# hjr37/diff-gaussian-rasterization

Hardware: AMD Instinct MI355X
Metric: Mviews/sec fwd+bwd @1080p, 500k Gaussians (higher is better)
Workload: dtype f32

## Files before the change

### diff-gaussian-rasterization_amd/csrc/api.hip

```cpp
#include <hip/hip_runtime.h>

#include <algorithm>
#include <string>

#include "../../include/dgr_hip.h"
#include "dgr_common.h"
#include "host_util.h"
#include "kernels.h"
#include "options.h"
#include "profile.h"
#include "status.h"

namespace dgr {
namespace {
thread_local std::string g_last_error = "";
}
void set_last_error(const std::string& text) { g_last_error = text; }
}

using namespace dgr;

namespace {

struct FwdCommon {
// ... 108 lines not shown
    return DGR_OK;
}

template <class A>
void blend_fwd_common(A& r, const FwdCommon& c, dgr::GeometryView geom, dgr::ImageView img, dgr::BinningView bin, ArmedReport* armed) {
    r.W = c.W; r.H = c.H; r.grid_x = dgr::tiles_x(c.W); r.grid_y = dgr::tiles_y(c.H);
    r.sched = img.tile_sched; r.ranges = img.ranges; r.sched_flag = img.cursor + 3; r.point_list = bin.point_list; r.rec = geom.rec; r.bg = c.background;
    r.out_color = c.out_color; r.out_depth = c.out_depth; r.n_contrib = img.n_contrib; r.status = img.status;
    r.rep = armed ? armed->rep : dgr::StatusReport{nullptr, 0u, nullptr};
}
int forward_blend(const FwdCommon& c, dgr::GeometryView geom, dgr::ImageView img, dgr::BinningView bin, hipStream_t st, bool full,
                  ArmedReport* armed = nullptr) {
    ScopedStage t(ST_RENDER_FWD, st);
    if (full) {
        dgr::RenderFwdFullArgs r{};
        blend_fwd_common(r, c, geom, img, bin, armed);
        r.out_uncertainty = c.out_alpha; r.n_valid = img.n_valid; r.first_contrib = img.first_contrib; r.final_T = img.final_T;
        HIP_TRY(dgr::launch_render_fwd_full(r, opt_alpha_mode(), st));
    } else {
        dgr::RenderFwdLightArgs r{};
        blend_fwd_common(r, c, geom, img, bin, armed);
        r.gt_depth = c.gt_depth; r.out_median = c.out_median_depth; r.out_alpha = c.out_alpha; r.out_depth_var = c.out_depth_var;
        r.gau_uncertainty = c.gau_uncertainty; r.gau_related_pixels = c.gau_related_pixels;
        HIP_TRY(dgr::launch_render_fwd_light(r, opt_alpha_mode(), st));
    }
    if (armed) armed->handed_over = true;
    return DGR_OK;
}

int check_common(const FwdCommon& c) {
    if (c.P < 0 || c.W <= 0 || c.H <= 0) { set_last_error("bad sizes"); return DGR_ERR_BAD_ARGUMENT; }
    if ((unsigned)c.P > DGR_ID_MASK) { set_last_error("more than 2^28 Gaussians"); return DGR_ERR_BAD_ARGUMENT; }
    if (c.P > 0 && !c.shs && !c.colors_precomp) { set_last_error("need SHs or precomputed colours"); return DGR_ERR_BAD_ARGUMENT; }
    if (c.P > 0 && !c.cov3D_precomp && (!c.scales || !c.rotations)) { set_last_error("need scale/rotation or cov3D"); return DGR_ERR_BAD_ARGUMENT; }
    if (dgr::tiles_x(c.W) > 65535 || dgr::tiles_y(c.H) > 65535 || (long long)c.W * c.H > (1ll << 30)) { set_last_error("image too large"); return DGR_ERR_BAD_ARGUMENT; }
    return DGR_OK;
}

inline int batch_stream_count(int n_views) {
    const int kmax = std::max(1, std::min(option(OPT_BATCH_STREAMS), DGR_BATCH_MAX_STREAMS));
    const int rounds = (n_views + kmax - 1) / kmax;
    return (n_views + rounds - 1) / rounds;
}
struct BatchStreams {
    int device = -1;
    hipStream_t helper[DGR_BATCH_MAX_STREAMS - 1] = {};
// ... 267 lines not shown
    s.ds = DetScratch{nullptr, nullptr, nullptr, 0};
    if (!scratch_clean) { ScopedStage t(ST_ZERO, st); HIP_TRY(dgr::launch_zero_fill(s.sc.acc, s.sc.zero_bytes, st)); }
    if (w.dL_dmean2D_abs) { ScopedStage t(ST_ZERO, st); HIP_TRY(dgr::launch_zero_floats(w.dL_dmean2D_abs, 3 * (size_t)P, st)); }
    if (det) {
        s.ds = carve_det_scratch(w.scratch, P, w.R);
        { ScopedStage t(ST_ZERO, st); HIP_TRY(dgr::launch_zero_fill(s.ds.rows, sizeof(float) * DGR_ACC_STRIDE * (size_t)w.R, st)); }
        HIP_TRY(dgr::launch_det_offsets(P, s.geom.rect, s.ds.blk, s.geom.goff, st));
    }
    return DGR_OK;
}

template <class A>
void blend_bwd_common(A& r, const BwdView& w, const float* bg, int W, int H, const BwdBufs& s, bool det) {
    r.W = W; r.H = H; r.grid_x = dgr::tiles_x(W); r.grid_y = dgr::tiles_y(H);
    r.sched = s.img.tile_sched; r.ranges = s.img.ranges; r.sched_flag = s.img.cursor + 3; r.point_list = (const uint32_t*)w.binning_buffer;
    r.rec = s.geom.rec; r.bg = bg; r.gt_depth = w.gt_depth; r.n_contrib = s.img.n_contrib; r.acc = s.sc.acc;
    if (det) { r.det_rows = s.ds.rows; r.det_rect = s.geom.rect; r.det_goff = s.geom.goff; r.det_R = (uint32_t)w.R; }
}
int blend_bwd_light(const BwdView& w, const dgr::PreprocessBwdArgs& b, const float* bg, const BwdBufs& s, bool det, bool complete,
                    hipStream_t st) {
    dgr::RenderBwdLightArgs r{};
    blend_bwd_common(r, w, bg, b.W, b.H, s, det);
    r.alphas = w.alphas; r.dL_dpix = w.dL_dpix; r.dL_dpix_depth = w.dL_dpix_depth; r.dL_dpix_median = w.dL_dpix_median_depth;
    r.dL_dpix_var = w.dL_dpix_depth_var; r.dL_dpix_silhouette = w.dL_dpix_silhouette;
    r.means3D = b.means3D; r.view = w.viewmatrix; r.track_off = b.track_off; r.map_off = complete ? 0 : b.map_off;
    ScopedStage t(ST_RENDER_BWD, st);
    if (w.dL_dmean2D_abs) HIP_TRY(dgr::launch_render_bwd_light_abs(r, w.dL_dmean2D_abs, opt_alpha_mode(), st));
    else HIP_TRY(dgr::launch_render_bwd_light(r, opt_alpha_mode(), st));
    return DGR_OK;
}
int blend_bwd_full(const BwdView& w, const dgr::PreprocessBwdArgs& b, const float* bg, const BwdBufs& s, bool det, hipStream_t st) {
    dgr::RenderBwdFullArgs r{};
    blend_bwd_common(r, w, bg, b.W, b.H, s, det);
    r.final_T = s.img.final_T; r.first_contrib = s.img.first_contrib;
    r.dL_dpix = w.dL_dpix; r.dL_depths = w.dL_depths; r.dL_duncertainties = w.dL_duncertainties;
    r.dL_dpix_silhouette = w.dL_dpix_silhouette;
    ScopedStage t(ST_RENDER_BWD, st);
    if (w.dL_dmean2D_abs) HIP_TRY(dgr::launch_render_bwd_full_abs(r, w.dL_dmean2D_abs, opt_alpha_mode(), st));
    else HIP_TRY(dgr::launch_render_bwd_full(r, opt_alpha_mode(), st, det));
    return DGR_OK;
}
int bwd_view_blend(const BwdView& w, const dgr::PreprocessBwdArgs& b, const float* bg, const BwdBufs& s, bool det, bool complete,
                   hipStream_t st) {
    const int rc = b.full_variant ? blend_bwd_full(w, b, bg, s, det, st) : blend_bwd_light(w, b, bg, s, det, complete, st);
    if (rc) return rc;
    if (det) HIP_TRY(dgr::launch_det_gather(b.P, s.geom.rect, s.geom.goff, s.ds.rows, (uint32_t)w.R, s.sc.acc, st));
    return DGR_OK;
// ... 534 lines not shown
```

### diff-gaussian-rasterization_amd/csrc/kernels.h

```cpp
#pragma once
#include <hip/hip_ext.h>
#include "dgr_common.h"

namespace dgr {

struct LaunchEvents {
    hipEvent_t start, stop;
    bool used;
};
extern thread_local LaunchEvents* g_launch_events;

template <typename K, typename... Args>
inline void launch(K kernel, dim3 grid, dim3 block, hipStream_t stream, Args... args) {
    LaunchEvents* ev = g_launch_events;
    if (ev && !ev->used) {
        ev->used = true;
        hipExtLaunchKernelGGL(kernel, grid, block, 0, stream, ev->start, ev->stop, 0, args...);
    } else {
        hipLaunchKernelGGL(kernel, grid, block, 0, stream, args...);
    }
}
template <typename K, typename... Args>
inline void launch_shmem(K kernel, dim3 grid, dim3 block, size_t shmem, hipStream_t stream, Args... args) {
    LaunchEvents* ev = g_launch_events;
// ... 110 lines not shown
    double* det_pose;
};
struct PreprocessBwdBatchArgs {
    PreprocessBwdArgs base;
    int V;
    BwdViewPart v[DGR_MAX_BATCH_VIEWS];
};

struct RenderFwdLightArgs {
    int W, H, grid_x, grid_y;
    const uint4* sched;
    const uint2* ranges;
    const uint32_t* sched_flag;
    uint32_t* point_list;
    const float4* rec;
    const float* bg;
    const float* gt_depth;
    float* out_color;
    float* out_depth;
    float* out_median;
    float* out_alpha;
    float* out_depth_var;
    uint32_t* n_contrib;
    float* gau_uncertainty;
    int* gau_related_pixels;
    StatusReport rep;
    const int* status;
};

struct RenderBwdLightArgs {
    int W, H, grid_x, grid_y;
    const uint4* sched;
    const uint2* ranges;
    const uint32_t* sched_flag;
    const uint32_t* point_list;
    const float4* rec;
    const float* bg;
    const float* gt_depth;
    const float* alphas;
    const uint32_t* n_contrib;
    const float* dL_dpix;
    const float* dL_dpix_depth;
    const float* dL_dpix_median;
    const float* dL_dpix_var;
    const float* dL_dpix_silhouette;
    const float* means3D;
    const float* view;
    float* acc;
    int track_off, map_off;
    float* det_rows;
    const ushort4* det_rect;
    const uint32_t* det_goff;
    uint32_t det_R;
};

struct RenderFwdFullArgs {
    int W, H, grid_x, grid_y;
    const uint4* sched;
    const uint2* ranges;
    const uint32_t* sched_flag;
    uint32_t* point_list;
    const float4* rec;
    const float* bg;
// ... 93 lines not shown
```

### diff-gaussian-rasterization_amd/csrc/render_common.h

```cpp
#pragma once
#include "dgr_common.h"
#include "kernels.h"
#include "wave_reduce.h"
#include "exact_math.h"

namespace dgr {

__device__ __forceinline__ uint4 blend_slot(const uint4* __restrict__ sched, const uint2* __restrict__ ranges,
                                            const uint32_t* __restrict__ sched_flag, int tiles, bool* overflowed = nullptr,
                                            bool* quadrant_lists = nullptr) {
    const int flag = __builtin_amdgcn_readfirstlane((int)*sched_flag);
    if (overflowed) *overflowed = (flag & 2) != 0;
    if (quadrant_lists) *quadrant_lists = (flag & 4) != 0;
    if (flag & 1) return sched[blockIdx.x];
    const int tile = xcd_contiguous((int)blockIdx.x, tiles);
    const uint2 r = ranges[tile];
    return make_uint4((uint32_t)tile, r.x, r.y, 0u);
}

__device__ __forceinline__ bool wave_any(bool p) { return __builtin_amdgcn_ballot_w64(p) != 0ull; }

namespace {

constexpr float LOG2E = 1.4426950408889634f, LN2 = 0.6931471805599453f;
// ... 6 lines not shown
    static constexpr float PSCALE = LOG2 ? LOG2E : 1.0f;
    static constexpr float PUNSCALE = LOG2 ? LN2 : 1.0f;
    static constexpr bool TABLE = (AM == ALPHA_GLIBC);
};
template <int AM, bool UNTESTED_ARG = false>
__device__ __forceinline__ float alpha_raw(float o, float p2, const uint64_t* tab) {
    if (AM == ALPHA_FAST) return o * __builtin_amdgcn_exp2f(p2);
    if (AM == ALPHA_GLIBC) return o * exp_glibc<UNTESTED_ARG>(p2, tab);
    return o * exp_p32<UNTESTED_ARG>(p2);
}
template <int AM>
__device__ __forceinline__ float t_div(float T, float om, float& inv) {
    if (AM == ALPHA_FAST) { inv = __builtin_amdgcn_rcpf(om); return T * inv; }
    return div_ref(T, om, inv);
}

template <int NB, typename LIST_T = unsigned short, int NLISTS = 4, bool KEEP_ID = true>
struct StagedT {
    typedef LIST_T list_t;
    static constexpr bool HAS_ID = KEEP_ID;
    static constexpr int SLOTS = NB;
    static constexpr int SENTINEL = NB;
    static constexpr int LIST_LD = NB + 8;
    float4 rec[2 * (NB + 1)];
    float4 rgbd[NB + 1];
    uint32_t id[KEEP_ID ? NB : 1];
    LIST_T list[NLISTS][LIST_LD];
    int cnt4[4][NLISTS];
};
using Staged = StagedT<DGR_TILE_PIX>;

template <bool HALF_CODES>
__device__ __forceinline__ unsigned reach_code(const float4& q0, const float4& q1, float l2, float tile_x0, float tile_y0);

template <int AM, bool HALF_CODES = false, class S>
__device__ __forceinline__ unsigned stage_one(S& s, int slot, uint32_t gid, const float4* __restrict__ rec,
                                              float tile_x0, float tile_y0) {
    const float4 q0 = rec[DGR_REC_STRIDE * (size_t)gid + 0];
    const float4 q1 = rec[DGR_REC_STRIDE * (size_t)gid + 1];
    const float4 q2 = rec[DGR_REC_STRIDE * (size_t)gid + 2];
    const float o = q0.w;
    const float l2 = __log2f(o * (255.0f / 15.0f));
    constexpr float PSCALE = AlphaPath<AM>::PSCALE;
    float lthr = (o > 0.f) ? (-l2 * (AlphaPath<AM>::LOG2 ? 1.0f : LN2) - 1.0e-4f) : 3.0e38f;
    float zword = __int_as_float(slot);
    if (HALF_CODES) {
// ... 42 lines not shown
}

__device__ __forceinline__ uint32_t pack4(uint32_t w) { return (w & 1u) | ((w >> 7) & 2u) | ((w >> 14) & 4u) | ((w >> 21) & 8u); }
__device__ __forceinline__ uint32_t tag_byte(uint32_t up, uint32_t lo) { return spread4(pack4(up)) | (spread4(pack4(lo)) << 1); }

template <int AM, int TAGS, class S>
__device__ __forceinline__ unsigned stage_tagged(S& s, int slot, uint32_t entry, const float4* __restrict__ rec,
                                                 const uint8_t* __restrict__ tag8) {
    constexpr float PSCALE = AlphaPath<AM>::PSCALE;
    unsigned code = (unsigned)*tag8;
    if (code == 0u) return 0u;
    if (TAGS == TAGS_BYTES_QUADRANT) code = fold8(code);
    const uint32_t gid = entry & ID_MASK;
    const float4 q0 = rec[DGR_REC_STRIDE * (size_t)gid + 0];
    const float4 q1 = rec[DGR_REC_STRIDE * (size_t)gid + 1];
    const float4 q2 = rec[DGR_REC_STRIDE * (size_t)gid + 2];
    s.rec[2 * slot] = make_float4(q0.x, q0.y, -0.5f * PSCALE * q1.x, -0.5f * PSCALE * q1.z);
    s.rec[2 * slot + 1] = make_float4(-PSCALE * q1.y, q0.w, __int_as_float(slot * 4), __int_as_float(slot * 16));
    s.rgbd[slot] = make_float4(q2.x, q2.y, q2.z, q0.z);
    s.id[slot] = gid;
    return code;
}

__device__ __forceinline__ int lanes_below(unsigned long long m) {
    return (int)__builtin_amdgcn_mbcnt_hi((unsigned)(m >> 32), __builtin_amdgcn_mbcnt_lo((unsigned)m, 0u));
}

template <class S>
__device__ __forceinline__ int build_lists(S& s, unsigned code, int tid, int wave, int lane) {
    typedef typename S::list_t LT;
    unsigned long long bal[4];
#pragma unroll
    for (int w = 0; w < 4; w++) {
        bal[w] = __ballot((code >> w) & 1u);
        if (lane == 0) s.cnt4[wave][w] = __popcll(bal[w]);
    }
    __syncthreads();
#pragma unroll
    for (int w = 0; w < 4; w++) {
        if ((code >> w) & 1u) {
            int base = 0;
            for (int sw = 0; sw < wave; sw++) base += s.cnt4[sw][w];
            s.list[w][base + lanes_below(bal[w])] = (LT)(tid * 32);
        }
    }
    const int n = __builtin_amdgcn_readfirstlane(s.cnt4[0][wave] + s.cnt4[1][wave] + s.cnt4[2][wave] + s.cnt4[3][wave]);
    __syncthreads();
    if (lane < 4) s.list[wave][n + lane] = (LT)(S::SENTINEL * 32);
    return n;
}

template <class S>
__device__ __forceinline__ int build_half_lists(S& s, unsigned code, int tid, int wave, int lane) {
    typedef typename S::list_t LT;
    unsigned long long bal[8];
#pragma unroll
    for (int l = 0; l < 8; l++) {
        bal[l] = __ballot((code >> l) & 1u);
        if (lane == 0) s.cnt4[wave][l] = __popcll(bal[l]);
    }
    __syncthreads();
    int before = 0, all = 0;
    if (lane < 8) {
#pragma unroll
        for (int sw = 0; sw < 4; sw++) {
            const int c = s.cnt4[sw][lane];
            before += sw < wave ? c : 0;
            all += c;
        }
    }
#pragma unroll
    for (int l = 0; l < 8; l++) {
        const int base = __builtin_amdgcn_readlane(before, l);
        if ((code >> l) & 1u) s.list[l][base + lanes_below(bal[l])] = (LT)(tid * 32);
    }
    const int l0 = 2 * wave;
    const int n0 = __builtin_amdgcn_readlane(all, l0), n1 = __builtin_amdgcn_readlane(all, l0 + 1);
    __syncthreads();
    const int n = max(n0, n1);
    for (int i = n0 + lane; i < n + 4; i += 64) s.list[l0][i] = (LT)(S::SENTINEL * 32);
    for (int i = n1 + lane; i < n + 4; i += 64) s.list[l0 + 1][i] = (LT)(S::SENTINEL * 32);
    return n;
}

template <class S>
__device__ __forceinline__ int build_paired_lists(S& s, unsigned code8, int tid, int wave, int lane, unsigned long long (&split)[2]) {
    typedef typename S::list_t LT;
    static_assert(sizeof(LT) == 4 && S::SLOTS <= 128, "paired lists: 32-bit entries, at most two ranks per lane");
    unsigned long long bal[4];
#pragma unroll
    for (int w = 0; w < 4; w++) {
        bal[w] = __ballot(((code8 >> (2 * w)) & 3u) != 0u);
        if (lane == 0) s.cnt4[wave][w] = __popcll(bal[w]);
    }
    __syncthreads();
    int before = 0, all = 0;
    if (lane < 4) {
#pragma unroll
        for (int sw = 0; sw < 4; sw++) {
            const int c = s.cnt4[sw][lane];
            before += sw < wave ? c : 0;
            all += c;
        }
    }
#pragma unroll
    for (int w = 0; w < 4; w++) {
        const unsigned t = (code8 >> (2 * w)) & 3u;
        const int base = __builtin_amdgcn_readlane(before, w);
        if (t != 0u) s.list[2 * w][base + lanes_below(bal[w])] = (LT)(tid * 32) | t;
    }
    const int n = __builtin_amdgcn_readlane(all, wave);
    __syncthreads();
    LT* const LU = s.list[2 * wave];
    LT* const LL = s.list[2 * wave + 1];
    if (n <= 64) {
        const bool have = lane < n;
        const unsigned e0 = have ? LU[lane] : 0u;
        const int t0 = (int)(e0 & 3u);
        const int tm1 = __builtin_amdgcn_update_dpp(0, t0, 0x138, 0xf, 0xf, true);
        const int tm2 = __builtin_amdgcn_update_dpp(0, tm1, 0x138, 0xf, 0xf, true);
        const int tp1 = __builtin_amdgcn_update_dpp(0, t0, 0x130, 0xf, 0xf, true);
        const int tp2 = __builtin_amdgcn_update_dpp(0, tp1, 0x130, 0xf, 0xf, true);
        const bool odd = (lane & 1) != 0;
        const bool a_self = odd ? (tm1 * t0 == 2) : (t0 * tp1 == 2);
        const bool a_side = odd ? (tp1 * tp2 == 2) : (tm2 * tm1 == 2);
        const bool p2 = !a_self && !a_side && (odd ? (t0 * tp1 == 2) : (tm1 * t0 == 2));
        const bool first = odd ? p2 : a_self, second = odd ? a_self : p2;
        const unsigned long long keep = __ballot(have && !second);
        const int steps = __popcll(keep);
        if (have) {
            const int st = lanes_below(keep) - (second ? 1 : 0);
            const LT o = e0 & ~3u;
            if (first || second) {
                (t0 == 1 ? LU : LL)[st] = o;
            } else {
                LU[st] = o;
                LL[st] = o;
            }
        }
        if (lane < 4) {
            LU[steps + lane] = (LT)(S::SENTINEL * 32);
            LL[steps + lane] = (LT)(S::SENTINEL * 32);
        }
        split[0] = __ballot(lane < steps && LU[lane] != LL[lane]);
        split[1] = 0ull;
        return steps;
    }
    const LT ea = lane < n ? LU[lane] : 0u, eb = lane + 64 < n ? LU[lane + 64] : 0u;
    if (lane < n) { LU[lane] = ea & ~3u; LL[lane] = ea & ~3u; }
    if (lane + 64 < n) { LU[lane + 64] = eb & ~3u; LL[lane + 64] = eb & ~3u; }
    if (lane < 4) {
        LU[n + lane] = (LT)(S::SENTINEL * 32);
        LL[n + lane] = (LT)(S::SENTINEL * 32);
    }
    split[0] = split[1] = 0ull;
    return n;
}

typedef float f2 __attribute__((ext_vector_type(2)));

template <int AM>
__device__ __forceinline__ float pair_p2(const float4& q0, const float4& q1, f2 pxy, f2& dxy) {
    const f2 g = {q0.x, q0.y}, ac = {q0.z, q0.w};
    dxy = g - pxy;
    if (AM == ALPHA_FAST) {
        const f2 m = ac * dxy;
        const float t = __builtin_fmaf(q1.x, dxy.y, m.x);
        return __builtin_fmaf(dxy.x, t, m.y * dxy.y);
    } else {
#pragma clang fp contract(off)
        const f2 m = (ac * dxy) * dxy;
        const float B = (q1.x * dxy.x) * dxy.y;
        return (m.x + m.y) + B;
    }
}

// ... 47 lines not shown
```

### diff-gaussian-rasterization_amd/csrc/render_light.hip

```cpp
#include "render_common.h"

namespace dgr {
namespace {

constexpr int FWD_UNROLL = 2;

template <bool HALVES>
struct StagedFwd {
    typedef StagedT<DGR_TILE_PIX, unsigned short, HALVES ? 8 : 4, !HALVES> staged_t;
    staged_t f;
    float unc[DGR_TILE_PIX];
    uint32_t cnt[DGR_TILE_PIX];
    uint32_t hit[DGR_TILE_PIX];
    uint64_t exptab[32];
};


template <class SF>
__device__ __forceinline__ void flush_slot(const SF& sf, const RenderFwdLightArgs& a, uint8_t* tag8, uint32_t pos0, int tid, bool staged) {
    if (!staged) return;
    uint32_t t8;
    if constexpr (!SF::staged_t::HAS_ID) {
        t8 = tag_byte(sf.hit[tid], __float_as_uint(sf.f.rec[2 * tid + 1].z));
    } else {
        t8 = spread4(pack4(sf.hit[tid])) * 3u;
    }
    tag8[pos0 + tid] = (uint8_t)t8;
    if (sf.cnt[tid] != 0u) {
        uint32_t gid;
        if constexpr (SF::staged_t::HAS_ID) gid = sf.f.id[tid];
        else gid = a.point_list[pos0 + tid];
        atomicAdd(&a.gau_uncertainty[gid], sf.unc[tid]);
        atomicAdd(&a.gau_related_pixels[gid], (int)sf.cnt[tid]);
    }
}

template <int AM, bool HALVES>
__device__ __forceinline__ void render_fwd_light_body(const RenderFwdLightArgs& a, StagedFwd<HALVES>& sf, const uint4 slot, const bool overflowed) {
    typename StagedFwd<HALVES>::staged_t& s = sf.f;
    const int tile = (int)slot.x;
    const int tx = tile % a.grid_x, ty = tile / a.grid_x;
    const int tid = threadIdx.x, wave = tid >> 6, lane = tid & 63;
    const int px = tx * DGR_BLOCK_X + (wave & 1) * 8 + (lane & 7);
    const int py = ty * DGR_BLOCK_Y + (wave >> 1) * 8 + (lane >> 3);
    const bool inside = px < a.W && py < a.H;
    const uint32_t pix_id = (uint32_t)a.W * (uint32_t)py + (uint32_t)px;
    const f2 pxy = {(float)px, (float)py};
    const float tile_x0 = (float)(tx * DGR_BLOCK_X), tile_y0 = (float)(ty * DGR_BLOCK_Y);
    const int my_list = HALVES ? 2 * wave + (lane >> 5) : wave;
    uint8_t* const tag8 = half_tags(a.point_list, a.sched_flag);
    unsigned char* const mark_base = (HALVES && lane >= 32) ? reinterpret_cast<unsigned char*>(&s.rec[1].z) + wave
                                                             : reinterpret_cast<unsigned char*>(sf.hit) + wave;
    const int mark_stride = (HALVES && lane >= 32) ? 32 : 4;

    const uint2 range = make_uint2(slot.y, slot.z);
    const int total = (int)(range.y - range.x);

    float T = 1.0f, C0 = 0.f, C1 = 0.f, C2 = 0.f, weight = 0.f, Dd = 0.f, D_median = 0.f;
    uint32_t last_contributor = 0;
    float ub = inside ? 0.f : -__builtin_inff();
    const float gt_px = inside ? a.gt_depth[pix_id] : 0.f;
    if (tid == 0) write_sentinel(s);
    if (AlphaPath<AM>::TABLE) exp_ref_table_fill(sf.exptab, tid);
    bool have_flush = false;
    int last_base = 0;

    for (int base = 0; base < total; base += DGR_TILE_PIX) {
        if (__syncthreads_and(ub < 0.f)) break;
        last_base = base;
        if (have_flush) flush_slot(sf, a, tag8, range.x + base - DGR_TILE_PIX, tid, true);
        sf.unc[tid] = 0.f;
        sf.cnt[tid] = 0u;
        sf.hit[tid] = 0u;
        have_flush = true;
        const int cnt = min(DGR_TILE_PIX, total - base);
        unsigned code = 0;
        if (tid < cnt) code = stage_one<AM, HALVES>(s, tid, a.point_list[range.x + base + tid], a.rec, tile_x0, tile_y0);
        const int n = HALVES ? build_half_lists(s, code, tid, wave, lane) : build_lists(s, code, tid, wave, lane);

        for (int k = 0; k < n; k += FWD_UNROLL) {
            float4 q0[FWD_UNROLL], q1[FWD_UNROLL];
            load2(s, my_list, k, q0, q1);
#pragma unroll
            for (int u = 0; u < FWD_UNROLL; u++) {
                f2 dxy;
                const float p2 = pair_p2<AM>(q0[u], q1[u], pxy, dxy);
                if ((p2 <= ub) & (p2 >= q1[u].w)) {
                  const float alpha = fminf(0.99f, alpha_raw<AM>(q1[u].y, p2, sf.exptab));
                  if (alpha >= ALPHA_MIN) {
#pragma clang fp contract(off)
                    const float test_T = T * (1.0f - alpha);
                    if (test_T < 0.0001f) {
                        ub = -__builtin_inff();
// ... 1 lines not shown
                        const int j = HALVES ? (__float_as_int(q1[u].w) & 0xFF) : __float_as_int(q1[u].z);
                        const float4 cd = s.rgbd[j];
                        mark_base[j * mark_stride] = 1;
                        const float w = alpha * T;
                        C0 = __builtin_fmaf(cd.x, w, C0); C1 = __builtin_fmaf(cd.y, w, C1); C2 = __builtin_fmaf(cd.z, w, C2);
                        weight = weight + w;
                        Dd = __builtin_fmaf(cd.w, w, Dd);
                        if (T > 0.5f && test_T < 0.5f) {
                            D_median = cd.w;
                            const float e = cd.w - gt_px;
                            atomicAdd(&sf.unc[j], e * e * w);
                            atomicAdd(&sf.cnt[j], 1u);
                        }
                        T = test_T;
                        last_contributor = (uint32_t)(base + j + 1);
                    }
                  }
                }
            }
            if (!wave_any(ub >= 0.f)) break;
        }
    }
    __syncthreads();
    if (have_flush) flush_slot(sf, a, tag8, range.x + last_base, tid, tid < total - last_base);
    for (int p = (have_flush ? last_base + DGR_TILE_PIX : 0) + tid; p < total; p += DGR_TILE_PIX) tag8[range.x + p] = 0;

    if (overflowed) {
        C0 = C1 = C2 = weight = Dd = D_median = __builtin_nanf("");
    }
    if (inside) {
        const uint32_t N = (uint32_t)a.W * (uint32_t)a.H;
        a.n_contrib[pix_id] = last_contributor;
        a.out_color[pix_id] = C0 + T * a.bg[0];
        a.out_color[N + pix_id] = C1 + T * a.bg[1];
        a.out_color[2 * N + pix_id] = C2 + T * a.bg[2];
        a.out_alpha[pix_id] = weight;
        a.out_depth[pix_id] = Dd;
        a.out_median[pix_id] = D_median;
        a.out_depth_var[pix_id] = 0.0f;
    }
}

template <int AM>
__global__ void __launch_bounds__(256, 8) render_fwd_light_kernel(RenderFwdLightArgs a) {
    __shared__ union { StagedFwd<true> h; StagedFwd<false> q; } sf;
    if (a.rep.host && blockIdx.x == 0 && threadIdx.x == 0) report_status(a.rep, a.status);
    bool overflowed, quadrant_lists;
    const uint4 slot = blend_slot(a.sched, a.ranges, a.sched_flag, a.grid_x * a.grid_y, &overflowed, &quadrant_lists);
    if (quadrant_lists) render_fwd_light_body<AM, false>(a, sf.q, slot, overflowed);
    else render_fwd_light_body<AM, true>(a, sf.h, slot, overflowed);
}

constexpr int NACC_LIGHT = 14;

template <bool DET, bool HALVES = false, bool ABS = false>
struct StagedBwd {
    static constexpr int NB = DET ? 64 : 128;
    static constexpr int LD = NB + 1;
    static constexpr int PLANE = NACC_LIGHT * LD;
    static constexpr int NACC = ABS ? NACC_LIGHT + 2 : NACC_LIGHT;
    typedef StagedT<NB, uint32_t, HALVES ? 8 : 4> staged_t;
    staged_t f;
    float acc[(DET ? 4 : 1) * PLANE + (ABS ? 2 * LD : 0)];
    uint32_t inst[DET ? NB : 1];
    int max_last;
    uint64_t exptab[32];
};

template <int AM, bool DO_MAP, bool DO_POSE, bool DET, bool LEAN, bool HALVES, bool ABS = false>
__device__ __forceinline__ void render_bwd_light_body(const RenderBwdLightArgs& a, StagedBwd<DET, HALVES, ABS>& sb, const uint4 slot,
                                                      float* __restrict__ abs_out = nullptr) {
    static_assert(!HALVES || !DET, "half-wave / paired lists: not with the deterministic kernel's planes (LDS)");
    static_assert(!ABS || (DO_MAP && !DET), "absgrad: the mapping backward, not the deterministic kernel");
    constexpr bool PAIRED = HALVES && DO_MAP;
    typedef StagedBwd<DET, HALVES, ABS> SB;
    constexpr int BWD_NB = SB::NB, BWD_LD = SB::LD;
    typename SB::staged_t& s = sb.f;
    const int tile = (int)slot.x;
    const int tx = tile % a.grid_x, ty = tile / a.grid_x;
    const int tid = threadIdx.x, wave = tid >> 6, lane = tid & 63;
    const int px = tx * DGR_BLOCK_X + (wave & 1) * 8 + (lane & 7);
    const int py = ty * DGR_BLOCK_Y + (wave >> 1) * 8 + (lane >> 3);
    const bool inside = px < a.W && py < a.H;
    const uint32_t pix_id = (uint32_t)a.W * (uint32_t)py + (uint32_t)px;
    const uint32_t N = (uint32_t)a.W * (uint32_t)a.H;
    const float pxf = (float)px, pyf = (float)py;
    const f2 pxy = {pxf, pyf};

    const uint2 range = make_uint2(slot.y, slot.z);
    const int last_contributor = inside ? (int)a.n_contrib[pix_id] : 0;

    if (tid == 0) {
        sb.max_last = 0;
        write_sentinel<true>(s);
    }
    if (AlphaPath<AM>::TABLE) exp_ref_table_fill(sb.exptab, tid);
    __syncthreads();
    {
        int v = last_contributor;
#pragma unroll
        for (int off = 32; off > 0; off >>= 1) v = max(v, __shfl_xor(v, off, 64));
        if (lane == 0) atomicMax(&sb.max_last, v);
    }
    __syncthreads();
    const int total = min((int)(range.y - range.x), sb.max_last);
    if (total <= 0) return;

    const float T_final = inside ? (1.0f - a.alphas[pix_id]) : 0.f;
    float T = T_final;
    float dpix0 = 0.f, dpix1 = 0.f, dpix2 = 0.f, dpix_depth = 0.f, dpix_median = 0.f, dpix_var = 0.f, gt_px = 0.f, dpix_sil = 0.f;
    if (inside) {
        dpix0 = __builtin_nontemporal_load(a.dL_dpix + pix_id);
        dpix1 = __builtin_nontemporal_load(a.dL_dpix + N + pix_id);
        dpix2 = __builtin_nontemporal_load(a.dL_dpix + 2 * N + pix_id);
        dpix_depth = __builtin_nontemporal_load(a.dL_dpix_depth + pix_id);
        if (a.dL_dpix_silhouette) dpix_sil = __builtin_nontemporal_load(a.dL_dpix_silhouette + pix_id);
        if (!LEAN) {
            if (a.dL_dpix_median) dpix_median = __builtin_nontemporal_load(a.dL_dpix_median + pix_id);
            if (a.dL_dpix_var) dpix_var = __builtin_nontemporal_load(a.dL_dpix_var + pix_id);
            gt_px = __builtin_nontemporal_load(a.gt_depth + pix_id);
        }
    }
    const float bg_term = -T_final * ((a.bg[0] * dpix0 + a.bg[1] * dpix1 + a.bg[2] * dpix2) - dpix_sil);
    const float ddelx_dx = 0.5f * a.W, ddely_dy = 0.5f * a.H;
    float S = 0.f;
    float mid_thr = 0.5f;
    int my_comp;
    if (DO_MAP) {
        const int c = (lane >= 48) ? 12 : wave_reduce12d_comp(lane);
        my_comp = ((lane & 3) != 0 || c > 11) ? -1 : (c == 10 ? (DO_POSE ? 13 : 10) : c == 11 ? (DO_POSE ? 10 : -1) : c);
    } else if (HALVES) {
        const int c = half_reduce3_comp(lane);
        my_comp = c == 0 ? 4 : c == 1 ? 5 : c == 2 ? 13 : -1;
    } else {
        const int c = wave_reduce4_comp(lane);
        my_comp = ((lane & 15) == 0 && c < 3) ? (c == 0 ? 4 : c == 1 ? 5 : 13) : -1;
    }
    const int my_list = HALVES ? 2 * wave + (lane >> 5) : wave;
    const uint8_t* const tag8 = half_tags(a.point_list, a.sched_flag);

    float* const my_acc = sb.acc + (DET ? wave * SB::PLANE : 0) + (my_comp >= 0 ? my_comp : 0) * BWD_LD;

    for (int hi = total; hi > 0; hi -= BWD_NB) {
        const int lo = max(0, hi - BWD_NB);
        const int cnt = hi - lo;
        __syncthreads();
        unsigned code = 0;
        if (tid < cnt) code = stage_tagged<AM, HALVES ? TAGS_BYTES_HALVES : TAGS_BYTES_QUADRANT>(s, tid, a.point_list[range.x + lo + tid], a.rec, tag8 + (range.x + lo + tid));
        if (!DET) {
#pragma unroll
            for (int k = 0; k < SB::NACC; k++)
                if (BWD_NB == DGR_TILE_PIX || tid < BWD_NB) sb.acc[k * BWD_LD + tid] = 0.f;
        }
        unsigned long long split[2] = {0ull, 0ull};
        const int n = PAIRED   ? build_paired_lists(s, code, tid, wave, lane, split)
                      : HALVES ? build_half_lists(s, code, tid, wave, lane)
                               : build_lists(s, code, tid, wave, lane);
        const int rel_last4 = 4 * (last_contributor - lo);

        constexpr int U = PAIRED ? 1 : 2;
        for (int k = ((n + U - 1) / U) * U - U; k >= 0; k -= U) {
            float4 q0[2], q1[2];
            if (U == 2) {
                load2(s, my_list, k, q0, q1);
            } else {
                const unsigned off = s.list[my_list][k];
                q0[0] = *reinterpret_cast<const float4*>(reinterpret_cast<const char*>(s.rec) + off);
                q1[0] = *reinterpret_cast<const float4*>(reinterpret_cast<const char*>(s.rec) + off + 16);
            }
#pragma unroll
            for (int u = U - 1; u >= 0; u--) {
                f2 dxy;
                const float p2 = pair_p2<AM>(q0[u], q1[u], pxy, dxy);
                const float dx = dxy.x, dy = dxy.y;
                const int j4 = __float_as_int(q1[u].z);
                const float oG = alpha_raw<AM, true>(q1[u].y, p2, sb.exptab);
                const bool valid = (j4 < rel_last4) & (p2 <= 0.0f) & !(oG < ALPHA_MIN);
                const float oGm = valid ? oG : 0.f;
                const float alpha = fminf(0.99f, oGm);
                const float4 cd = *reinterpret_cast<const float4*>(reinterpret_cast<const char*>(s.rgbd) + __float_as_int(q1[u].w));
                const float om = 1.f - alpha;
                float inv;
                T = t_div<AM>(T, om, inv);
                const float w = alpha * T;
                const float e = cd.w - gt_px;
                const float X = LEAN ? cd.x * dpix0 + cd.y * dpix1 + cd.z * dpix2 + cd.w * dpix_depth
                                     : cd.x * dpix0 + cd.y * dpix1 + cd.z * dpix2 + cd.w * dpix_depth + (e * e) * dpix_var;
                const float dL_dalpha = (X - S) * T + bg_term * inv;
                S = alpha * X + om * S;
                const float qq = oGm * dL_dalpha;
                const float qdx = qq * dx, qdy = qq * dy;
                const float wd = w * dpix_depth;
                float tot;
                if (DO_MAP) {
                    float gmed = 0.f;
                    if (!LEAN) {
                        const bool fire = valid & (T > mid_thr);
                        gmed = fire ? dpix_median : 0.f;
                        mid_thr = fire ? __builtin_inff() : mid_thr;
                    }
                    float g[12];
                    g[0] = w * dpix0;
                    g[1] = w * dpix1;
// ... 51 lines not shown
        if (DET && tid < BWD_NB) {
            uint32_t row = ~0u;
            if (code != 0u) {
#pragma unroll
                for (int k = 0; k < NACC_LIGHT; k++) {
                    const bool delivered = DO_MAP ? (k <= 9 || k == 10 || (DO_POSE && k == 13)) : (k == 4 || k == 5 || k == 13);
                    float v = 0.f;
                    if (delivered) {
#pragma unroll
                        for (int w = 0; w < 4; w++)
                            if ((code >> w) & 1u) v += sb.acc[w * SB::PLANE + k * BWD_LD + tid];
                    }
                    sb.acc[k * BWD_LD + tid] = v;
                }
                const uint32_t gid = s.id[tid];
                const ushort4 rc = a.det_rect[gid];
                row = a.det_goff[gid] + (uint32_t)(ty - (int)rc.y) * (uint32_t)(rc.z - rc.x) + (uint32_t)(tx - (int)rc.x);
            }
            sb.inst[tid] = row;
        }
        if (DET) __syncthreads();
        if (code != 0u) {
            constexpr float UN = AlphaPath<AM>::PUNSCALE;
            const float4 r0 = s.rec[2 * tid], r1 = s.rec[2 * tid + 1];
            const float ca = r0.z * (-2.f * UN), cb = r1.x * (-UN), cc = r0.w * (-2.f * UN);
            const float Sx = sb.acc[4 * BWD_LD + tid], Sy = sb.acc[5 * BWD_LD + tid];
            sb.acc[4 * BWD_LD + tid] = -(ca * Sx + cb * Sy) * ddelx_dx;
            sb.acc[5 * BWD_LD + tid] = -(cc * Sy + cb * Sx) * ddely_dy;
            if (ABS) {
                const float ax = sb.acc[NACC_LIGHT * BWD_LD + tid] * ddelx_dx, ay = sb.acc[(NACC_LIGHT + 1) * BWD_LD + tid] * ddely_dy;
                const size_t gid = s.id[tid];
                if (ax != 0.f) atomicAdd(abs_out + 3 * gid, ax);
                if (ay != 0.f) atomicAdd(abs_out + 3 * gid + 1, ay);
            }
            if (DO_MAP) {
                sb.acc[6 * BWD_LD + tid] *= -0.5f;
                sb.acc[7 * BWD_LD + tid] *= -0.5f;
                sb.acc[8 * BWD_LD + tid] *= -0.5f;
                sb.acc[9 * BWD_LD + tid] *= __builtin_amdgcn_rcpf(r1.y);
            }
        }
        __syncthreads();
        if (DET) {
            const int comp = tid & 15;
            for (int r = tid >> 4; r < cnt; r += 16) {
                const uint32_t row = sb.inst[r];
                if (row < a.det_R && comp < NACC_LIGHT) a.det_rows[(size_t)row * DGR_ACC_STRIDE + comp] = sb.acc[comp * BWD_LD + r];
// ... 282 lines not shown
```

### diff-gaussian-rasterization_amd/csrc/state_export.hip

```cpp
#include <hip/hip_runtime.h>

#include <string>

#include "dgr_common.h"
#include "host_util.h"

namespace {

enum ExportKind { EX_MEANS2D, EX_CONIC_OPACITY, EX_RGB, EX_CLAMPED, EX_TILES_TOUCHED, EX_KEYS };

__global__ void export_geom_kernel(int kind, int P, dgr::GeometryView g, void* dst) {
    const int i = blockIdx.x * 256 + threadIdx.x;
    if (i >= P) return;
    const bool vis = g.radii[i] > 0;
    switch (kind) {
        case EX_MEANS2D: {
            const float4 q = g.rec[DGR_REC_STRIDE * (size_t)i];
            ((float2*)dst)[i] = vis ? make_float2(q.x, q.y) : make_float2(0, 0);
        } break;
        case EX_CONIC_OPACITY: {
            const float4 q0 = g.rec[DGR_REC_STRIDE * (size_t)i], q1 = g.rec[DGR_REC_STRIDE * (size_t)i + 1];
            ((float4*)dst)[i] = vis ? make_float4(q1.x, q1.y, q1.z, q0.w) : make_float4(0, 0, 0, 0);
        } break;
        case EX_RGB: {
// ... 59 lines not shown
    if (n == "depths") return copy(g.depths, 4 * (size_t)P) ? -1 : P;
    if (n == "radii") return copy(g.radii, 4 * (size_t)P) ? -1 : P;
    if (n == "means2D") return geomk(EX_MEANS2D) ? -1 : 2L * P;
    if (n == "conic_opacity") return geomk(EX_CONIC_OPACITY) ? -1 : 4L * P;
    if (n == "rgb") return geomk(EX_RGB) ? -1 : 3L * P;
    if (n == "clamped") return geomk(EX_CLAMPED) ? -1 : 3L * P;
    if (n == "tiles_touched") return geomk(EX_TILES_TOUCHED) ? -1 : P;
    if (n == "point_list" || n == "contribution_tags" || n == "half_tags") {
        if (num_rendered > 0) {
            const dim3 grid((num_rendered + 255) / 256);
            if (n == "point_list")
                hipLaunchKernelGGL(export_point_list_kernel, grid, dim3(256), 0, st, bin.point_list, (uint32_t*)dst, num_rendered);
            else
                hipLaunchKernelGGL(export_tag_bytes_kernel, grid, dim3(256), 0, st, bin.pair_cov, (uint8_t*)dst, num_rendered, n == "half_tags" ? 1 : 0);
            if (hipGetLastError() != hipSuccess) return -1;
        }
        return num_rendered;
    }
    if (n == "keys") {
        hipLaunchKernelGGL(export_keys_kernel, dim3((unsigned)tiles), dim3(256), 0, st, img, bin, g, (uint64_t*)dst);
        if (hipGetLastError() != hipSuccess) return -1;
        return num_rendered;
    }
    if (n == "ranges") return copy(img.ranges, 8 * tiles) ? -1 : (long)(2 * tiles);
    if (n == "tile_sched") return copy(img.tile_sched, 16 * tiles) ? -1 : (long)(4 * tiles);
    if (n == "sched_flag") return copy(img.cursor + 3, 4) ? -1 : 1L;
    if (n == "n_contrib") return copy(img.n_contrib, 4 * N) ? -1 : (long)N;
    if (n == "n_valid") return copy(img.n_valid, 4 * N) ? -1 : (long)N;
    if (n == "final_T") return copy(img.final_T, 4 * N) ? -1 : (long)N;
    dgr::set_last_error("unknown state array: " + n);
    return -1;
}

}
```

Baseline: 0.002635.

## Compact live Gaussian-pixel pairs in light forward for a dense backward pass

The light forward renderer now stream-compacts each tile's contributing entries (nonzero tag byte) into a per-tile live list of (gid, position<<8|tag) pairs. It records the live count per tile, reusing the pair_keys buffer and tile_count array. The light backward iterates only over this compacted list, dropping the max-last-contributor reduction and the tag byte gather. It stages colour/depth inline in a 48-byte record instead of a separate rgbd array. This trades an extra ballot, syncthreads and global write per flush in forward, plus larger shared records, for less backward work on culled entries.

```diff
diff --git a/diff-gaussian-rasterization_amd/csrc/api.hip b/diff-gaussian-rasterization_amd/csrc/api.hip
--- a/diff-gaussian-rasterization_amd/csrc/api.hip
+++ b/diff-gaussian-rasterization_amd/csrc/api.hip
@@ -154,6 +154,7 @@
         blend_fwd_common(r, c, geom, img, bin, armed);
         r.gt_depth = c.gt_depth; r.out_median = c.out_median_depth; r.out_alpha = c.out_alpha; r.out_depth_var = c.out_depth_var;
         r.gau_uncertainty = c.gau_uncertainty; r.gau_related_pixels = c.gau_related_pixels;
+        r.live_counts = img.tile_count;
         HIP_TRY(dgr::launch_render_fwd_light(r, opt_alpha_mode(), st));
     }
     if (armed) armed->handed_over = true;
@@ -467,7 +468,7 @@
     dgr::RenderBwdLightArgs r{};
     blend_bwd_common(r, w, bg, b.W, b.H, s, det);
     r.alphas = w.alphas; r.dL_dpix = w.dL_dpix; r.dL_dpix_depth = w.dL_dpix_depth; r.dL_dpix_median = w.dL_dpix_median_depth;
-    r.dL_dpix_var = w.dL_dpix_depth_var; r.dL_dpix_silhouette = w.dL_dpix_silhouette;
+    r.dL_dpix_var = w.dL_dpix_depth_var; r.dL_dpix_silhouette = w.dL_dpix_silhouette; r.live_counts = s.img.tile_count;
     r.means3D = b.means3D; r.view = w.viewmatrix; r.track_off = b.track_off; r.map_off = complete ? 0 : b.map_off;
     ScopedStage t(ST_RENDER_BWD, st);
     if (w.dL_dmean2D_abs) HIP_TRY(dgr::launch_render_bwd_light_abs(r, w.dL_dmean2D_abs, opt_alpha_mode(), st));
diff --git a/diff-gaussian-rasterization_amd/csrc/kernels.h b/diff-gaussian-rasterization_amd/csrc/kernels.h
--- a/diff-gaussian-rasterization_amd/csrc/kernels.h
+++ b/diff-gaussian-rasterization_amd/csrc/kernels.h
@@ -156,6 +156,7 @@
     float* out_alpha;
     float* out_depth_var;
     uint32_t* n_contrib;
+    uint32_t* live_counts;
     float* gau_uncertainty;
     int* gau_related_pixels;
     StatusReport rep;
@@ -173,6 +174,7 @@
     const float* gt_depth;
     const float* alphas;
     const uint32_t* n_contrib;
+    const uint32_t* live_counts;
     const float* dL_dpix;
     const float* dL_dpix_depth;
     const float* dL_dpix_median;
diff --git a/diff-gaussian-rasterization_amd/csrc/render_common.h b/diff-gaussian-rasterization_amd/csrc/render_common.h
--- a/diff-gaussian-rasterization_amd/csrc/render_common.h
+++ b/diff-gaussian-rasterization_amd/csrc/render_common.h
@@ -52,6 +52,7 @@
     static constexpr int SLOTS = NB;
     static constexpr int SENTINEL = NB;
     static constexpr int LIST_LD = NB + 8;
+    static constexpr int REC_BYTES = 32;
     float4 rec[2 * (NB + 1)];
     float4 rgbd[NB + 1];
     uint32_t id[KEEP_ID ? NB : 1];
@@ -140,6 +141,47 @@
     return code;
 }
 
+__device__ __forceinline__ uint2* live_list(const uint32_t* point_list, const uint32_t* sched_flag) {
+    return reinterpret_cast<uint2*>(carve_binning(reinterpret_cast<char*>(const_cast<uint32_t*>(point_list)), (size_t)sched_flag[-1]).pair_keys);
+}
+
+template <int NB, int NLISTS = 4>
+struct StagedLiveT {
+    typedef uint32_t list_t;
+    static constexpr bool HAS_ID = true;
+    static constexpr int SLOTS = NB;
+    static constexpr int SENTINEL = NB;
+    static constexpr int LIST_LD = NB + 8;
+    static constexpr int REC_BYTES = 48;
+    float4 rec[3 * (NB + 1)];
+    uint32_t id[NB];
+    uint32_t list[NLISTS][LIST_LD];
+    int cnt4[4][NLISTS];
+};
+
+template <int AM, bool QUADRANT, class S>
+__device__ __forceinline__ unsigned stage_live(S& s, int slot, uint2 e, const float4* __restrict__ rec) {
+    constexpr float PSCALE = AlphaPath<AM>::PSCALE;
+    unsigned code = e.y & 0xFFu;
+    if (QUADRANT) code = fold8(code);
+    const uint32_t gid = e.x & ID_MASK;
+    const float4 q0 = rec[DGR_REC_STRIDE * (size_t)gid + 0];
+    const float4 q1 = rec[DGR_REC_STRIDE * (size_t)gid + 1];
+    const float4 q2 = rec[DGR_REC_STRIDE * (size_t)gid + 2];
+    s.rec[3 * slot] = make_float4(q0.x, q0.y, -0.5f * PSCALE * q1.x, -0.5f * PSCALE * q1.z);
+    s.rec[3 * slot + 1] = make_float4(-PSCALE * q1.y, q0.w, __int_as_float(slot * 4), __int_as_float((int)(e.y >> 8)));
+    s.rec[3 * slot + 2] = make_float4(q2.x, q2.y, q2.z, q0.z);
+    s.id[slot] = gid;
+    return code;
+}
+template <class S>
+__device__ __forceinline__ void write_sentinel_live(S& s) {
+    constexpr int NB = S::SLOTS;
+    s.rec[3 * NB] = make_float4(0.f, 0.f, 0.f, 0.f);
+    s.rec[3 * NB + 1] = make_float4(0.f, 0.f, __int_as_float(NB * 4), __int_as_float(0x7fffffff));
+    s.rec[3 * NB + 2] = make_float4(0.f, 0.f, 0.f, 0.f);
+}
+
 __device__ __forceinline__ int lanes_below(unsigned long long m) {
     return (int)__builtin_amdgcn_mbcnt_hi((unsigned)(m >> 32), __builtin_amdgcn_mbcnt_lo((unsigned)m, 0u));
 }
@@ -159,12 +201,12 @@
         if ((code >> w) & 1u) {
             int base = 0;
             for (int sw = 0; sw < wave; sw++) base += s.cnt4[sw][w];
-            s.list[w][base + lanes_below(bal[w])] = (LT)(tid * 32);
+            s.list[w][base + lanes_below(bal[w])] = (LT)(tid * S::REC_BYTES);
         }
     }
     const int n = __builtin_amdgcn_readfirstlane(s.cnt4[0][wave] + s.cnt4[1][wave] + s.cnt4[2][wave] + s.cnt4[3][wave]);
     __syncthreads();
-    if (lane < 4) s.list[wave][n + lane] = (LT)(S::SENTINEL * 32);
+    if (lane < 4) s.list[wave][n + lane] = (LT)(S::SENTINEL * S::REC_BYTES);
     return n;
 }
 
@@ -190,14 +232,14 @@
 #pragma unroll
     for (int l = 0; l < 8; l++) {
         const int base = __builtin_amdgcn_readlane(before, l);
-        if ((code >> l) & 1u) s.list[l][base + lanes_below(bal[l])] = (LT)(tid * 32);
+        if ((code >> l) & 1u) s.list[l][base + lanes_below(bal[l])] = (LT)(tid * S::REC_BYTES);
     }
     const int l0 = 2 * wave;
     const int n0 = __builtin_amdgcn_readlane(all, l0), n1 = __builtin_amdgcn_readlane(all, l0 + 1);
     __syncthreads();
     const int n = max(n0, n1);
-    for (int i = n0 + lane; i < n + 4; i += 64) s.list[l0][i] = (LT)(S::SENTINEL * 32);
-    for (int i = n1 + lane; i < n + 4; i += 64) s.list[l0 + 1][i] = (LT)(S::SENTINEL * 32);
+    for (int i = n0 + lane; i < n + 4; i += 64) s.list[l0][i] = (LT)(S::SENTINEL * S::REC_BYTES);
+    for (int i = n1 + lane; i < n + 4; i += 64) s.list[l0 + 1][i] = (LT)(S::SENTINEL * S::REC_BYTES);
     return n;
 }
 
@@ -225,7 +267,7 @@
     for (int w = 0; w < 4; w++) {
         const unsigned t = (code8 >> (2 * w)) & 3u;
         const int base = __builtin_amdgcn_readlane(before, w);
-        if (t != 0u) s.list[2 * w][base + lanes_below(bal[w])] = (LT)(tid * 32) | t;
+        if (t != 0u) s.list[2 * w][base + lanes_below(bal[w])] = (LT)(tid * S::REC_BYTES) | t;
     }
     const int n = __builtin_amdgcn_readlane(all, wave);
     __syncthreads();
@@ -257,8 +299,8 @@
             }
         }
         if (lane < 4) {
-            LU[steps + lane] = (LT)(S::SENTINEL * 32);
-            LL[steps + lane] = (LT)(S::SENTINEL * 32);
+            LU[steps + lane] = (LT)(S::SENTINEL * S::REC_BYTES);
+            LL[steps + lane] = (LT)(S::SENTINEL * S::REC_BYTES);
         }
         split[0] = __ballot(lane < steps && LU[lane] != LL[lane]);
         split[1] = 0ull;
@@ -268,8 +310,8 @@
     if (lane < n) { LU[lane] = ea & ~3u; LL[lane] = ea & ~3u; }
     if (lane + 64 < n) { LU[lane + 64] = eb & ~3u; LL[lane + 64] = eb & ~3u; }
     if (lane < 4) {
-        LU[n + lane] = (LT)(S::SENTINEL * 32);
-        LL[n + lane] = (LT)(S::SENTINEL * 32);
+        LU[n + lane] = (LT)(S::SENTINEL * S::REC_BYTES);
+        LL[n + lane] = (LT)(S::SENTINEL * S::REC_BYTES);
     }
     split[0] = split[1] = 0ull;
     return n;
diff --git a/diff-gaussian-rasterization_amd/csrc/render_light.hip b/diff-gaussian-rasterization_amd/csrc/render_light.hip
--- a/diff-gaussian-rasterization_amd/csrc/render_light.hip
+++ b/diff-gaussian-rasterization_amd/csrc/render_light.hip
@@ -12,27 +12,39 @@
     float unc[DGR_TILE_PIX];
     uint32_t cnt[DGR_TILE_PIX];
     uint32_t hit[DGR_TILE_PIX];
+    alignas(16) uint32_t live4[4];
     uint64_t exptab[32];
 };
 
-
 template <class SF>
-__device__ __forceinline__ void flush_slot(const SF& sf, const RenderFwdLightArgs& a, uint8_t* tag8, uint32_t pos0, int tid, bool staged) {
-    if (!staged) return;
-    uint32_t t8;
-    if constexpr (!SF::staged_t::HAS_ID) {
-        t8 = tag_byte(sf.hit[tid], __float_as_uint(sf.f.rec[2 * tid + 1].z));
-    } else {
-        t8 = spread4(pack4(sf.hit[tid])) * 3u;
-    }
-    tag8[pos0 + tid] = (uint8_t)t8;
-    if (sf.cnt[tid] != 0u) {
+__device__ __forceinline__ uint32_t flush_slot(SF& sf, const RenderFwdLightArgs& a, uint8_t* tag8, uint2* live, uint32_t list0, uint32_t pos0,
+                                               uint32_t live_base, int tid, bool staged) {
+    uint32_t t8 = 0u;
+    if (staged) {
+        if constexpr (!SF::staged_t::HAS_ID) {
+            t8 = tag_byte(sf.hit[tid], __float_as_uint(sf.f.rec[2 * tid + 1].z));
+        } else {
+            t8 = spread4(pack4(sf.hit[tid])) * 3u;
+        }
+        tag8[list0 + pos0 + tid] = (uint8_t)t8;
+    }
+    const unsigned long long bal = __ballot(t8 != 0u);
+    if ((tid & 63) == 0) sf.live4[tid >> 6] = (uint32_t)__popcll(bal);
+    __syncthreads();
+    const uint4 c = *reinterpret_cast<const uint4*>(sf.live4);
+    if (t8 != 0u) {
+        const int wave = tid >> 6;
+        const uint32_t before = (wave > 0 ? c.x : 0u) + (wave > 1 ? c.y : 0u) + (wave > 2 ? c.z : 0u);
         uint32_t gid;
         if constexpr (SF::staged_t::HAS_ID) gid = sf.f.id[tid];
-        else gid = a.point_list[pos0 + tid];
-        atomicAdd(&a.gau_uncertainty[gid], sf.unc[tid]);
-        atomicAdd(&a.gau_related_pixels[gid], (int)sf.cnt[tid]);
-    }
+        else gid = a.point_list[list0 + pos0 + tid];
+        live[list0 + live_base + before + (uint32_t)lanes_below(bal)] = make_uint2(gid, ((pos0 + (uint32_t)tid) << 8) | t8);
+        if (sf.cnt[tid] != 0u) {
+            atomicAdd(&a.gau_uncertainty[gid], sf.unc[tid]);
+            atomicAdd(&a.gau_related_pixels[gid], (int)sf.cnt[tid]);
+        }
+    }
+    return live_base + (uint32_t)__builtin_amdgcn_readfirstlane((int)(c.x + c.y + c.z + c.w));
 }
 
 template <int AM, bool HALVES>
@@ -49,6 +61,8 @@
     const float tile_x0 = (float)(tx * DGR_BLOCK_X), tile_y0 = (float)(ty * DGR_BLOCK_Y);
     const int my_list = HALVES ? 2 * wave + (lane >> 5) : wave;
     uint8_t* const tag8 = half_tags(a.point_list, a.sched_flag);
+    uint2* const live = live_list(a.point_list, a.sched_flag);
+    uint32_t live_base = 0;
     unsigned char* const mark_base = (HALVES && lane >= 32) ? reinterpret_cast<unsigned char*>(&s.rec[1].z) + wave
                                                              : reinterpret_cast<unsigned char*>(sf.hit) + wave;
     const int mark_stride = (HALVES && lane >= 32) ? 32 : 4;
@@ -68,7 +82,7 @@
     for (int base = 0; base < total; base += DGR_TILE_PIX) {
         if (__syncthreads_and(ub < 0.f)) break;
         last_base = base;
-        if (have_flush) flush_slot(sf, a, tag8, range.x + base - DGR_TILE_PIX, tid, true);
+        if (have_flush) live_base = flush_slot(sf, a, tag8, live, range.x, (uint32_t)(base - DGR_TILE_PIX), live_base, tid, true);
         sf.unc[tid] = 0.f;
         sf.cnt[tid] = 0u;
         sf.hit[tid] = 0u;
@@ -116,7 +130,8 @@
         }
     }
     __syncthreads();
-    if (have_flush) flush_slot(sf, a, tag8, range.x + last_base, tid, tid < total - last_base);
+    if (have_flush) live_base = flush_slot(sf, a, tag8, live, range.x, (uint32_t)last_base, live_base, tid, tid < total - last_base);
+    if (tid == 0) a.live_counts[tile] = live_base;
     for (int p = (have_flush ? last_base + DGR_TILE_PIX : 0) + tid; p < total; p += DGR_TILE_PIX) tag8[range.x + p] = 0;
 
     if (overflowed) {
@@ -153,11 +168,10 @@
     static constexpr int LD = NB + 1;
     static constexpr int PLANE = NACC_LIGHT * LD;
     static constexpr int NACC = ABS ? NACC_LIGHT + 2 : NACC_LIGHT;
-    typedef StagedT<NB, uint32_t, HALVES ? 8 : 4> staged_t;
+    typedef StagedLiveT<NB, HALVES ? 8 : 4> staged_t;
     staged_t f;
     float acc[(DET ? 4 : 1) * PLANE + (ABS ? 2 * LD : 0)];
     uint32_t inst[DET ? NB : 1];
-    int max_last;
     uint64_t exptab[32];
 };
 
@@ -181,24 +195,13 @@
     const float pxf = (float)px, pyf = (float)py;
     const f2 pxy = {pxf, pyf};
 
-    const uint2 range = make_uint2(slot.y, slot.z);
+    const int total = __builtin_amdgcn_readfirstlane((int)a.live_counts[tile]);
+    if (total <= 0) return;
+    const uint2* const live = live_list(a.point_list, a.sched_flag) + slot.y;
     const int last_contributor = inside ? (int)a.n_contrib[pix_id] : 0;
 
-    if (tid == 0) {
-        sb.max_last = 0;
-        write_sentinel<true>(s);
-    }
+    if (tid == 0) write_sentinel_live(s);
     if (AlphaPath<AM>::TABLE) exp_ref_table_fill(sb.exptab, tid);
-    __syncthreads();
-    {
-        int v = last_contributor;
-#pragma unroll
-        for (int off = 32; off > 0; off >>= 1) v = max(v, __shfl_xor(v, off, 64));
-        if (lane == 0) atomicMax(&sb.max_last, v);
-    }
-    __syncthreads();
-    const int total = min((int)(range.y - range.x), sb.max_last);
-    if (total <= 0) return;
 
     const float T_final = inside ? (1.0f - a.alphas[pix_id]) : 0.f;
     float T = T_final;
@@ -231,7 +234,6 @@
         my_comp = ((lane & 15) == 0 && c < 3) ? (c == 0 ? 4 : c == 1 ? 5 : 13) : -1;
     }
     const int my_list = HALVES ? 2 * wave + (lane >> 5) : wave;
-    const uint8_t* const tag8 = half_tags(a.point_list, a.sched_flag);
 
     float* const my_acc = sb.acc + (DET ? wave * SB::PLANE : 0) + (my_comp >= 0 ? my_comp : 0) * BWD_LD;
 
@@ -240,7 +242,7 @@
         const int cnt = hi - lo;
         __syncthreads();
         unsigned code = 0;
-        if (tid < cnt) code = stage_tagged<AM, HALVES ? TAGS_BYTES_HALVES : TAGS_BYTES_QUADRANT>(s, tid, a.point_list[range.x + lo + tid], a.rec, tag8 + (range.x + lo + tid));
+        if (tid < cnt) code = stage_live<AM, !HALVES>(s, tid, live[lo + tid], a.rec);
         if (!DET) {
 #pragma unroll
             for (int k = 0; k < SB::NACC; k++)
@@ -250,17 +252,22 @@
         const int n = PAIRED   ? build_paired_lists(s, code, tid, wave, lane, split)
                       : HALVES ? build_half_lists(s, code, tid, wave, lane)
                                : build_lists(s, code, tid, wave, lane);
-        const int rel_last4 = 4 * (last_contributor - lo);
 
         constexpr int U = PAIRED ? 1 : 2;
         for (int k = ((n + U - 1) / U) * U - U; k >= 0; k -= U) {
             float4 q0[2], q1[2];
+            unsigned off[2];
             if (U == 2) {
-                load2(s, my_list, k, q0, q1);
+                const uint2 pk = *reinterpret_cast<const uint2*>(&s.list[my_list][k]);
+                off[0] = pk.x;
+                off[1] = pk.y;
             } else {
-                const unsigned off = s.list[my_list][k];
-                q0[0] = *reinterpret_cast<const float4*>(reinterpret_cast<const char*>(s.rec) + off);
-                q1[0] = *reinterpret_cast<const float4*>(reinterpret_cast<const char*>(s.rec) + off + 16);
+                off[0] = off[1] = s.list[my_list][k];
+            }
+#pragma unroll
+            for (int u = 0; u < U; u++) {
+                q0[u] = *reinterpret_cast<const float4*>(reinterpret_cast<const char*>(s.rec) + off[u]);
+                q1[u] = *reinterpret_cast<const float4*>(reinterpret_cast<const char*>(s.rec) + off[u] + 16);
             }
 #pragma unroll
             for (int u = U - 1; u >= 0; u--) {
@@ -269,10 +276,10 @@
                 const float dx = dxy.x, dy = dxy.y;
                 const int j4 = __float_as_int(q1[u].z);
                 const float oG = alpha_raw<AM, true>(q1[u].y, p2, sb.exptab);
-                const bool valid = (j4 < rel_last4) & (p2 <= 0.0f) & !(oG < ALPHA_MIN);
+                const bool valid = (__float_as_int(q1[u].w) < last_contributor) & (p2 <= 0.0f) & !(oG < ALPHA_MIN);
                 const float oGm = valid ? oG : 0.f;
                 const float alpha = fminf(0.99f, oGm);
-                const float4 cd = *reinterpret_cast<const float4*>(reinterpret_cast<const char*>(s.rgbd) + __float_as_int(q1[u].w));
+                const float4 cd = *reinterpret_cast<const float4*>(reinterpret_cast<const char*>(s.rec) + off[u] + 32);
                 const float om = 1.f - alpha;
                 float inv;
                 T = t_div<AM>(T, om, inv);
@@ -370,7 +377,7 @@
         if (DET) __syncthreads();
         if (code != 0u) {
             constexpr float UN = AlphaPath<AM>::PUNSCALE;
-            const float4 r0 = s.rec[2 * tid], r1 = s.rec[2 * tid + 1];
+            const float4 r0 = s.rec[3 * tid], r1 = s.rec[3 * tid + 1];
             const float ca = r0.z * (-2.f * UN), cb = r1.x * (-UN), cc = r0.w * (-2.f * UN);
             const float Sx = sb.acc[4 * BWD_LD + tid], Sy = sb.acc[5 * BWD_LD + tid];
             sb.acc[4 * BWD_LD + tid] = -(ca * Sx + cb * Sy) * ddelx_dx;
diff --git a/diff-gaussian-rasterization_amd/csrc/state_export.hip b/diff-gaussian-rasterization_amd/csrc/state_export.hip
--- a/diff-gaussian-rasterization_amd/csrc/state_export.hip
+++ b/diff-gaussian-rasterization_amd/csrc/state_export.hip
@@ -105,6 +105,8 @@
         if (hipGetLastError() != hipSuccess) return -1;
         return num_rendered;
     }
+    if (n == "live_list") return copy(bin.pair_keys, 8 * (size_t)num_rendered) ? -1 : 2L * num_rendered;
+    if (n == "live_counts") return copy(img.tile_count, 4 * tiles) ? -1 : (long)tiles;
     if (n == "ranges") return copy(img.ranges, 8 * tiles) ? -1 : (long)(2 * tiles);
     if (n == "tile_sched") return copy(img.tile_sched, 16 * tiles) ? -1 : (long)(4 * tiles);
     if (n == "sched_flag") return copy(img.cursor + 3, 4) ? -1 : 1L;
```

After: 0.002736, median of 6. 3.8% higher.
